# jamie8johnson/cqs

Measured on AMD Instinct MI355X. Metric: queries/sec @k=20 (brute-force cosine scan + top-k, 768-d fp32), higher is better.
Workload: dtype f32; 1 GPU; BASELINE configs[1]: 1000000 x 768 fp32 unit vectors, 1 query per step, brute-force cosine top-20; mode=single, rows_per_gpu=1000000, total_rows=1000000, dim=768, k=20, parallelism=single GPU, ranks_seen=1

## Files before the change

### cqs_amd/csrc/f32_score.h

```cpp
#pragma once
#include "scan_device.h"

namespace cqs {

template <int NCH, bool NT = false>
__device__ __forceinline__ void f32_row_fragments(const float* rp, uint32_t dim, uint32_t lane, f4 (&x)[NCH]) {
#pragma unroll
    for (int c = 0; c < NCH; ++c) {
        const uint32_t idx = (uint32_t)c * 256u + lane * 4u;
        const uint32_t off = idx < dim ? idx : dim - 4u;
        if (NT) x[c] = __builtin_nontemporal_load((const f4*)(rp + off));
        else x[c] = *(const f4*)(rp + off);
    }
}

template <int NCH>
__device__ __forceinline__ void f32_fragments(const float* rp, const float* qp, uint32_t dim, uint32_t lane, f4 (&x)[NCH],
                                              f4 (&qv)[NCH]) {
#pragma unroll
    for (int c = 0; c < NCH; ++c) {
        const uint32_t idx = (uint32_t)c * 256u + lane * 4u;
        const bool in = idx < dim;
        const uint32_t off = in ? idx : dim - 4u;
        x[c] = *(const f4*)(rp + off);
        const f4 v = *(const f4*)(qp + off);
        qv[c] = in ? v : (f4)(0.f);
    }
}

template <int NCH>
__device__ __forceinline__ float f32_dot_chain(const f4 (&x)[NCH], const f4 (&qv)[NCH]) {
    f2 acc2 = (f2)(0.f);
#pragma unroll
    for (int c = 0; c < NCH; ++c) {
        const f2 xlo = __builtin_shufflevector(x[c], x[c], 0, 1);
        const f2 xhi = __builtin_shufflevector(x[c], x[c], 2, 3);
        acc2 = __builtin_elementwise_fma(xlo, __builtin_shufflevector(qv[c], qv[c], 0, 1), acc2);
        acc2 = __builtin_elementwise_fma(xhi, __builtin_shufflevector(qv[c], qv[c], 2, 3), acc2);
    }
    float s = acc2.x + acc2.y;
#pragma unroll
    for (int m = 32; m >= 1; m >>= 1) s += __shfl_xor(s, m, 64);
    return s;
}

__device__ __forceinline__ bool f32_emit(float& s, uint32_t mode, float thr) {
    bool keep = __builtin_fabsf(s) <= 3.4028234664e38f;
    if (keep && mode == 1u) {
        s = s < 0.f ? 0.f : (s > 1.f ? 1.f : s);
        keep = s >= thr;
    }
    return keep;
}

}
```

### cqs_amd/csrc/index.hip

```cpp
#include <hip/hip_runtime.h>

#include <algorithm>
#include <cstdio>
#include <cstdlib>
#include <cstring>
#include <new>

#include "abi_guard.h"
#include "roctx.h"
#include "index_internal.h"
#include "scan_bf16.h"
#include "scan_i8.h"
#include "search_host.h"

using cqs::kMaxK;
using cqs::kRowsPerBlock;

namespace cqs_idx {

uint64_t pad_rows(uint64_t n) { return (n + kRowsPerBlock - 1) / kRowsPerBlock * kRowsPerBlock; }

int32_t fail(cqs_hip_index* idx, int32_t code, const char* what, hipError_t e) {
    char buf[512];
    if (e != hipSuccess)
// ... 148 lines not shown
    return CQS_HIP_OK;
}

void free_keep_tab(cqs_hip_index* x) {
    hipFree(x->d_keep_tab);
    hipHostFree(x->h_keep_tab);
    x->d_keep_tab = nullptr; x->h_keep_tab = nullptr; x->keep_tab_stride = 0;
}

bool ensure_keep_tab(cqs_hip_index* x) {
    const uint64_t cap = x->cap_rows > x->n ? x->cap_rows : x->n;
    const uint64_t stride = (cap + 31) / 32;
    if (x->d_keep_tab && x->keep_tab_stride >= stride) return true;
    if (stride > 0xFFFFFFFFull || quiesce(x) != hipSuccess) return false;
    free_keep_tab(x);
    const size_t bytes = (size_t)kCombineCap * stride * sizeof(uint32_t);
    if (hipMalloc(&x->d_keep_tab, bytes) != hipSuccess || hipHostMalloc(&x->h_keep_tab, bytes, hipHostMallocDefault) != hipSuccess) {
        (void)hipGetLastError();
        free_keep_tab(x);
        return false;
    }
    x->keep_tab_stride = stride;
    return true;
}

void read_combine_env(cqs_hip_index* x) {
    if (const char* ce = getenv("CQS_HIP_COMBINE")) x->combine = ce[0] != '0';
    if (const char* cf = getenv("CQS_HIP_COMBINE_FILTERED")) x->combine_filtered = cf[0] != '0';
    if (const char* ct = getenv("CQS_HIP_COMBINE_TAGGED")) x->combine_tagged = ct[0] != '0';
    x->cq.wait_us = cqs_combine::wait_us_from_env();
    if (const char* cb = getenv("CQS_HIP_COMBINE_BITS")) x->combine_relaxed = cb[0] == 'r';
}

int32_t create_common(uint64_t n, uint32_t dim, uint32_t metric, int32_t device, uint64_t row_base,
                      cqs_hip_index** out, cqs_hip_index** made) {
    if (!out) return CQS_HIP_ERR_INVALID;
    *out = nullptr;
    if (!cqs::scan_dim_supported(dim) || metric > CQS_HIP_METRIC_DOT) return CQS_HIP_ERR_INVALID;
    if (n + row_base > 0xFFFFFFFEull) return CQS_HIP_ERR_INVALID;
    int cnt = 0;
    if (hipGetDeviceCount(&cnt) != hipSuccess || cnt <= 0) return CQS_HIP_ERR_NO_DEVICE;
    if (device < 0 || device >= cnt) return CQS_HIP_ERR_INVALID;
    cqs_hip_index* x = new (std::nothrow) cqs_hip_index();
    if (!x) return CQS_HIP_ERR_NOMEM;
    x->device = device; x->n = n; x->dim = dim; x->metric = metric; x->row_base = row_base;
    if (hipSetDevice(device) != hipSuccess || hipStreamCreateWithFlags(&x->stream, hipStreamNonBlocking) != hipSuccess ||
        hipEventCreateWithFlags(&x->done, hipEventDisableTiming) != hipSuccess) {
        if (x->stream) hipStreamDestroy(x->stream);
        delete x;
        return CQS_HIP_ERR_DEVICE;
    }
    read_combine_env(x);
    if (getenv("CQS_HIP_DEBUG_STAMPS")) {
        const size_t bytes = (16 + 2 * cqs::kDbgWaves) * sizeof(unsigned long long);
        if (hipMalloc(&x->d_dbg, bytes) == hipSuccess) (void)hipMemset(x->d_dbg, 0, bytes);
    }
    hipDeviceProp_t prop;
    if (hipGetDeviceProperties(&prop, device) == hipSuccess && prop.multiProcessorCount > 0)
        x->n_cu = (uint32_t)prop.multiProcessorCount;
    *made = x;
    return CQS_HIP_OK;
}

}

using namespace cqs_idx;

extern "C" {

const char* cqs_hip_version(void) CQS_ABI_TRY { return "cqs-hip 0.1.0 (gfx950)"; } CQS_ABI_CATCH_VAL("cqs-hip")

int32_t cqs_hip_device_count(void) CQS_ABI_TRY {
    int cnt = 0;
    if (hipGetDeviceCount(&cnt) != hipSuccess) return 0;
    return cnt;
} CQS_ABI_CATCH_NOHANDLE

int32_t cqs_hip_device_mem(int32_t device, uint64_t* free_bytes, uint64_t* total_bytes) CQS_ABI_TRY {
    if (hipSetDevice(device) != hipSuccess) return CQS_HIP_ERR_NO_DEVICE;
    size_t f = 0, t = 0;
    if (hipMemGetInfo(&f, &t) != hipSuccess) return CQS_HIP_ERR_DEVICE;
    if (free_bytes) *free_bytes = f;
    if (total_bytes) *total_bytes = t;
    return CQS_HIP_OK;
} CQS_ABI_CATCH_NOHANDLE

}

int32_t cqs_idx::create_owned(const float* rows, uint64_t n, uint32_t dim, uint32_t metric, int32_t device,
                              uint64_t row_base, cqs_hip_index** out) {
    if (n > 0 && !rows) return CQS_HIP_ERR_INVALID;
    cqs_hip_index* x = nullptr;
    int32_t rc = create_common(n, dim, metric, device, row_base, out, &x);
    if (rc != CQS_HIP_OK) return rc;
    x->cap_rows = n ? n : 1;
    hipError_t e = hipMalloc(&x->d_rows, (size_t)x->cap_rows * dim * sizeof(float));
    if (e == hipSuccess && n)
        e = hipMemcpyAsync(x->d_rows, rows, (size_t)n * dim * sizeof(float), hipMemcpyHostToDevice, x->stream);
    if (e == hipSuccess) e = hipStreamSynchronize(x->stream);
    if (e != hipSuccess) {
        cqs_hip_index_destroy(x);
        return e == hipErrorOutOfMemory ? CQS_HIP_ERR_NOMEM : CQS_HIP_ERR_DEVICE;
    }
    *out = x;
    return CQS_HIP_OK;
}

// ... 466 lines not shown
```

### cqs_amd/csrc/index_shadow.hip

```cpp
#include <cstdlib>
#include <cstring>
#include <new>

#include "abi_guard.h"
#include "index_internal.h"
#include "scan_bf16.h"
#include "scan_fallback.h"
#include "scan_i8.h"

namespace cqs_idx {

constexpr uint64_t kShadowAutoBytes = 1ull << 30;
constexpr uint64_t kShadowFreeMinBytes = 4ull << 30;
constexpr double kShadowFreeFrac = 0.10;
constexpr uint32_t kStatWords = 12, kStatCounts = 3, kStatI8 = 5, kStatI8Counts = 8, kStatPrefix = 10;

struct Shadow {
    uint16_t* d_bf16 = nullptr;
    uint64_t cap = 0;
    int8_t* d_i8 = nullptr;
    float* d_i8_scale = nullptr;
    double r8 = 0.0, norm8 = 0.0;
    double r = 0.0;
    double norm = 0.0;
    unsigned long long* d_stats = nullptr;
    uint64_t* d_ekeys = nullptr;
    uint32_t* d_cert = nullptr;
    float* d_bq = nullptr;
    uint32_t* d_tickets = nullptr;
    uint64_t* d_fb_lists = nullptr;
    uint32_t* d_fb_tickets = nullptr;
    bool fb_one_launch = true;
    bool tail_prefix = true;
    uint8_t i8_groups = 2;
    uint32_t* h_cert = nullptr;
    uint32_t* h_cert_dev = nullptr;
};

static void shadow_device_counts(cqs_hip_index* x, uint32_t first, uint64_t* certified, uint64_t* fallbacks) {
    unsigned long long c[2];
    if (!x->shadow || !x->shadow->d_stats || quiesce(x) != hipSuccess) return;
    hipError_t e = hipMemcpyAsync(c, x->shadow->d_stats + first, sizeof c, hipMemcpyDeviceToHost, x->stream);
    if (e == hipSuccess) e = hipStreamSynchronize(x->stream);
    if (e != hipSuccess) { (void)hipGetLastError(); return; }
    *certified += c[0];
    *fallbacks += c[1];
}

static void i8_free(Shadow* s) {
    hipFree(s->d_i8); hipFree(s->d_i8_scale);
    s->d_i8 = nullptr; s->d_i8_scale = nullptr;
}

void shadow_free(cqs_hip_index* x) {
    Shadow* s = x->shadow;
    if (!s) return;
    uint64_t c = 0, f = 0;
    shadow_device_counts(x, kStatCounts, &c, &f);
    x->stat_certified.fetch_add(c, std::memory_order_relaxed);
    x->stat_fallbacks.fetch_add(f, std::memory_order_relaxed);
    c = f = 0;
    shadow_device_counts(x, kStatI8Counts, &c, &f);
    x->stat_i8_certified.fetch_add(c, std::memory_order_relaxed);
    x->stat_i8_fallbacks.fetch_add(f, std::memory_order_relaxed);
    i8_free(s);
    hipFree(s->d_bf16); hipFree(s->d_stats); hipFree(s->d_ekeys);
    hipFree(s->d_cert); hipFree(s->d_bq); hipFree(s->d_tickets); hipFree(s->d_fb_lists); hipFree(s->d_fb_tickets);
    hipHostFree(s->h_cert);
    delete s;
    x->shadow = nullptr;
}

ShadowBuffers shadow_buffers(const cqs_hip_index* x) {
    const Shadow* s = x->shadow;
    return s ? ShadowBuffers{s->d_bf16, s->d_i8, s->d_i8_scale} : ShadowBuffers{nullptr, nullptr, nullptr};
}

static int32_t shadow_convert(cqs_hip_index* x, uint64_t row0, bool* outlier) {
    Shadow* s = x->shadow;
    HIP_TRY(x, hipMemsetAsync(s->d_stats + 2, 0, sizeof(unsigned long long), x->stream));
    HIP_TRY(x, cqs::launch_shadow_build(x->d_rows, s->d_bf16, row0, x->n - row0, x->dim, cqs::shadow_gamma(x->dim),
                                        s->d_stats, x->stream));
    unsigned long long st[3];
    HIP_TRY(x, hipMemcpyAsync(st, s->d_stats, sizeof st, hipMemcpyDeviceToHost, x->stream));
    HIP_TRY(x, hipStreamSynchronize(x->stream));
    double r, m;
// ... 93 lines not shown
                hipFree(n8);
                i8_free(s);
                x->last_error = "extend: no device memory to grow the int8 copy of the shadow; int8 copy turned off";
            } else {
                e = hipMemcpyAsync(n8, s->d_i8, (size_t)n_old * x->dim, hipMemcpyDeviceToDevice, x->stream);
                if (e == hipSuccess) e = hipMemcpyAsync(ns, s->d_i8_scale, (size_t)n_old * sizeof(float), hipMemcpyDeviceToDevice, x->stream);
                if (e == hipSuccess) e = hipStreamSynchronize(x->stream);
                if (e != hipSuccess) { hipFree(n8); hipFree(ns); return fail(x, CQS_HIP_ERR_DEVICE, "extend: int8 copy", e); }
                i8_free(s);
                s->d_i8 = n8;
                s->d_i8_scale = ns;
            }
        }
        s->cap = x->cap_rows;
    }
    bool outlier = false;
    int32_t rc = shadow_convert(x, n_old, &outlier);
    if (rc == CQS_HIP_OK && s->d_i8 && !outlier) rc = i8_convert(x, n_old);
    if (rc != CQS_HIP_OK) return rc;
    if (outlier) {
        shadow_free(x);
        x->last_error = "extend: a new row has a component of magnitude >= 2^64; bf16 shadow turned off";
    }
    return CQS_HIP_OK;
}

static bool dim_ok(uint32_t dim) { return dim % 8u == 0u && dim <= cqs::kShadowMaxDim; }
static const char* const kDimRule = ": dim must be a multiple of 8 and <= 2048";

static int32_t shadow_enable(cqs_hip_index* x, const char* what) {
    std::string pre(what);
    if (!dim_ok(x->dim)) return fail(x, CQS_HIP_ERR_INVALID, (pre + kDimRule).c_str());
    if (x->shadow) return CQS_HIP_OK;
    auto oom = [&](hipError_t e) { (void)hipGetLastError(); shadow_free(x); return fail(x, CQS_HIP_ERR_NOMEM, (pre + ": allocation").c_str(), e); };
    Shadow* s = x->shadow = new (std::nothrow) Shadow();
    if (!s) return oom(hipErrorOutOfMemory);
    const uint64_t cap = x->cap_rows ? x->cap_rows : 1;
    hipError_t e;
    if ((e = hipMalloc(&s->d_bf16, (size_t)cap * x->dim * sizeof(uint16_t))) != hipSuccess) return oom(e);
    s->cap = cap;
    unsigned long long* stats = nullptr;
    if ((e = hipMalloc(&stats, kStatWords * sizeof(unsigned long long))) != hipSuccess) return oom(e);
    if ((e = hipMemsetAsync(stats, 0, kStatWords * sizeof(unsigned long long), x->stream)) != hipSuccess) { hipFree(stats); return oom(e); }
    s->d_stats = stats;
    if ((e = hipMalloc(&s->d_ekeys, (size_t)cqs::kShadowMaxQ * (cqs::kMaxK - 1) * sizeof(uint64_t))) != hipSuccess) return oom(e);
    if ((e = hipMalloc(&s->d_cert, (size_t)cqs::kShadowMaxQ * sizeof(uint32_t))) != hipSuccess) return oom(e);
    if ((e = hipMalloc(&s->d_bq, (size_t)cqs::kShadowMaxQ * sizeof(float))) != hipSuccess) return oom(e);
    if ((e = hipMalloc(&s->d_tickets, (size_t)cqs::kShadowMaxQ * sizeof(uint32_t))) != hipSuccess) return oom(e);
    if ((e = hipMemsetAsync(s->d_tickets, 0, (size_t)cqs::kShadowMaxQ * sizeof(uint32_t), x->stream)) != hipSuccess) return oom(e);
    const char* fb_env = getenv("CQS_HIP_FALLBACK_ONE_LAUNCH");
    s->fb_one_launch = !(fb_env && fb_env[0] == '0');
    const char* tp_env = getenv("CQS_HIP_TAIL_PREFIX");
    s->tail_prefix = !(tp_env && tp_env[0] == '0');
    const char* ig_env = getenv("CQS_HIP_I8_GROUPS");
    s->i8_groups = ig_env && ig_env[0] == '0' ? 0 : (ig_env && ig_env[0] == '1' ? 1 : 2);
    if ((e = hipMalloc(&s->d_fb_lists, cqs::f32_topk_fallback_words(x->n_cu) * sizeof(uint64_t))) != hipSuccess) return oom(e);
    if ((e = hipMalloc(&s->d_fb_tickets, (size_t)cqs::kMaxGemvQ * sizeof(uint32_t))) != hipSuccess) return oom(e);
    if ((e = hipMemsetAsync(s->d_fb_tickets, 0, (size_t)cqs::kMaxGemvQ * sizeof(uint32_t), x->stream)) != hipSuccess) return oom(e);
    if ((e = hipHostMalloc(&s->h_cert, (size_t)cqs::kShadowMaxQ * sizeof(uint32_t), hipHostMallocDefault)) != hipSuccess) return oom(e);
    if (hipHostGetDevicePointer((void**)&s->h_cert_dev, s->h_cert, 0) != hipSuccess) {
        (void)hipGetLastError();
        s->h_cert_dev = nullptr;
    }
    bool outlier = false;
    const int32_t rc = shadow_convert(x, 0, &outlier);
    if (rc != CQS_HIP_OK) { shadow_free(x); return rc; }
    if (outlier) {
        shadow_free(x);
        return fail(x, CQS_HIP_ERR_INVALID, (pre + ": a finite row has a component of magnitude >= 2^64").c_str());
    }
    return CQS_HIP_OK;
}

static bool i8_dim_ok(uint32_t dim) { return cqs::i8_dim_ok(dim); }
static const char* const kI8DimRule = ": dim must be a multiple of 16 and <= 2048";
static int32_t i8_auto(cqs_hip_index* x) {
    Shadow* s = x->shadow;
    if (!s || s->d_i8) return CQS_HIP_OK;
    const char* env = getenv("CQS_HIP_SCAN_I8");
    if (env && env[0] == '0') return CQS_HIP_OK;
    if (!(env && env[0] == '1') && x->n * x->dim * sizeof(float) < kShadowAutoBytes) return CQS_HIP_OK;
    const std::string pre("int8 copy of the shadow not built (the bf16 copy serves every block)");
    if (!i8_dim_ok(x->dim)) { x->last_error = pre + kI8DimRule; return CQS_HIP_OK; }
    size_t free_b = 0, total_b = 0;
    if (hipMemGetInfo(&free_b, &total_b) != hipSuccess) {
        (void)hipGetLastError();
        x->last_error = pre + ": hipMemGetInfo failed";
        return CQS_HIP_OK;
    }
    const uint64_t need = i8_bytes(s->cap, x->dim);
    const uint64_t frac = (uint64_t)(kShadowFreeFrac * (double)total_b);
    const uint64_t reserve = frac > kShadowFreeMinBytes ? frac : kShadowFreeMinBytes;
    bool built = false;
    if (free_b >= need && free_b - need >= reserve) {
        const int32_t rc = i8_enable(x, &built);
        if (rc != CQS_HIP_OK) return rc;
    }
    if (!built) x->last_error = pre + ": the device would keep less than max(4 GiB, 10 %) of its memory free with both copies";
    return CQS_HIP_OK;
}

int32_t shadow_auto(cqs_hip_index* x) {
    const char* env = getenv("CQS_HIP_SCAN_BF16");
    if (env && env[0] == '0') return CQS_HIP_OK;
    const bool any_size = env && env[0] == '1';
    const uint64_t f32_bytes = x->n * x->dim * sizeof(float);
// ... 15 lines not shown
    const uint64_t need = cap * x->dim * sizeof(uint16_t) + (cqs::kMaxK + 2ull) * cqs::kShadowMaxQ * sizeof(uint64_t) +
                          cqs::f32_topk_fallback_words(x->n_cu) * sizeof(uint64_t);
    const uint64_t frac = (uint64_t)(kShadowFreeFrac * (double)total_b);
    const uint64_t reserve = frac > kShadowFreeMinBytes ? frac : kShadowFreeMinBytes;
    if (free_b < need || free_b - need < reserve) {
        x->last_error = "bf16 shadow not built: the device would keep less than max(4 GiB, 10 %) of its memory free";
        return CQS_HIP_OK;
    }
    int32_t rc = shadow_enable(x, "bf16 shadow not built");
    if (rc == CQS_HIP_OK) rc = i8_auto(x);
    return rc == CQS_HIP_ERR_DEVICE ? rc : CQS_HIP_OK;
}

bool shadow_takes(const cqs_hip_index* x, uint32_t b, uint32_t k, bool gemv_only) {
    return x->shadow && b <= cqs::kShadowMaxQ && (gemv_only || !cqs::use_mfma(b, x->dim)) && cqs::shadow_kprime(k) >= k;
}

bool shadow_uses_i8(const cqs_hip_index* x, uint32_t b, uint32_t k) {
    return x->shadow && x->shadow->d_i8 && b <= cqs::kI8MaxQ && cqs::i8_k_ok(k);
}

static uint32_t shadow_group_tasks(const cqs_hip_index* x, bool i8, uint32_t kp) {
    const Shadow* s = x->shadow;
    if (!i8 || s->i8_groups == 0) return 1u;
    if (s->i8_groups == 1) return cqs::kMaxGroupTasks;
    const uint64_t kk = (uint64_t)kp + 1u;
    return 4u * kk * kk <= pad_rows(x->n) ? cqs::kMaxGroupTasks : 1u;
}

int32_t shadow_pass(cqs_hip_index* x, const float* d_q, uint32_t nb, uint32_t k, const uint32_t* d_keep, uint32_t mode,
                    float threshold, uint64_t* out_keys, uint32_t* out_counts, hipStream_t st, const uint32_t** device_gate,
                    const KeepTab* tab) {
    const Shadow* s = x->shadow;
    uint32_t* const cert = device_gate || !s->h_cert_dev ? s->d_cert : s->h_cert_dev;
    if (device_gate) *device_gate = cert;
    if (device_gate) HIP_TRY(x, order_after_last(x, st));
    const bool i8 = shadow_uses_i8(x, nb, k);
    const uint32_t kp = i8 ? cqs::i8_kprime(k) : cqs::shadow_kprime(k);
    const double r_max = i8 ? s->r8 : s->r, norm_max = i8 ? s->norm8 : s->norm;
    const bool bound_first = mode == CQS_HIP_MODE_PIPELINE;
    if (bound_first) {
        if (i8) HIP_TRY(x, cqs::launch_i8_bound(d_q, nb, x->dim, r_max, norm_max, s->d_bq, st));
        else HIP_TRY(x, cqs::launch_shadow_bound(d_q, nb, x->dim, r_max, norm_max, s->d_bq, st));
    }
    cqs::ScanArgs a = scan_args(x, d_q, nb, kp + 1u, d_keep, mode, threshold, i8 ? sizeof(int8_t) : sizeof(uint16_t), true, nullptr, nullptr, tab);
    a.group_tasks = shadow_group_tasks(x, i8, kp);
    const ShadowRows rows{i8 ? nullptr : s->d_bf16, i8 ? s->d_i8 : nullptr, s->d_i8_scale, s->d_bq};
    const int32_t rc = scan_select(x, a, st, &rows, nullptr, nullptr);
    if (rc == CQS_HIP_OK)
        HIP_TRY(x, cqs::launch_rescore_certify(a, (uint32_t)x->row_base, k, kp, bound_first ? 0u : (i8 ? 2u : 1u), r_max, norm_max,
                                               s->d_bq, s->d_tickets, s->d_ekeys, out_keys, out_counts, cert,
                                               device_gate ? s->d_stats + kStatCounts : nullptr,
                                               device_gate && i8 ? s->d_stats + kStatI8Counts : nullptr, s->tail_prefix,
                                               s->d_stats + kStatPrefix, x->d_dbg, st));
    return rc;
}

int32_t shadow_fallback(cqs_hip_index* x, const float* d_q, uint32_t nb, uint32_t k, const uint32_t* d_keep, uint32_t mode,
                        float threshold, uint64_t* out_keys, uint32_t* out_counts, hipStream_t st, const uint32_t* gate,
                        bool* taken) {
    const Shadow* s = x->shadow;
    *taken = false;
    if (!s || !gate || !s->fb_one_launch) return CQS_HIP_OK;
    const cqs::ScanArgs a = scan_args(x, d_q, nb, k, d_keep, mode, threshold, sizeof(float), false, nullptr, gate);
    if (!cqs::f32_topk_fallback_takes(a)) return CQS_HIP_OK;
    HIP_TRY(x, cqs::launch_f32_topk_fallback(a, (uint32_t)x->row_base, gate, s->d_fb_lists, s->d_fb_tickets, out_keys, out_counts, st));
    HIP_TRY(x, record_done(x, st));
    *taken = true;
    return CQS_HIP_OK;
}

hipError_t shadow_verdicts(cqs_hip_index* x, uint32_t nb, const uint32_t** h_cert) {
    const Shadow* s = x->shadow;
    *h_cert = s->h_cert;
    return s->h_cert_dev ? hipSuccess : hipMemcpyAsync(s->h_cert, s->d_cert, (size_t)nb * sizeof(uint32_t), hipMemcpyDeviceToHost, x->stream);
}

}

using namespace cqs_idx;

extern "C" {

int32_t cqs_hip_index_set_bf16_scan(cqs_hip_index* x, int32_t enable) CQS_ABI_TRY {
    if (!x || x->sh) return CQS_HIP_ERR_INVALID;
    std::lock_guard<std::mutex> g(x->mu);
    if (x->poisoned.load(std::memory_order_acquire)) return CQS_HIP_ERR_POISONED;
    HIP_TRY(x, hipSetDevice(x->device));
    HIP_TRY(x, quiesce(x));
    if (!enable) { shadow_free(x); return CQS_HIP_OK; }
    if (x->borrow) return fail(x, CQS_HIP_ERR_INVALID, "set_bf16_scan: index borrows its rows (they may change under the bound)");
    const int32_t rc = shadow_enable(x, "set_bf16_scan");
    return rc == CQS_HIP_OK ? i8_auto(x) : rc;
} CQS_ABI_CATCH(x)

void cqs_hip_index_bf16_stats(const cqs_hip_index* x, uint64_t* bytes, uint64_t* certified, uint64_t* fallbacks) CQS_ABI_TRY {
    uint64_t by = 0, c = 0, f = 0;
    if (x && !x->sh) {
        cqs_hip_index* m = const_cast<cqs_hip_index*>(x);
        std::lock_guard<std::mutex> g(m->mu);
        by = m->shadow ? m->shadow->cap * m->dim * sizeof(uint16_t) : 0;
        c = m->stat_certified.load(std::memory_order_relaxed);
        f = m->stat_fallbacks.load(std::memory_order_relaxed);
        if (m->shadow && hipSetDevice(m->device) == hipSuccess) shadow_device_counts(m, kStatCounts, &c, &f);
    }
    if (bytes) *bytes = by;
// ... 58 lines not shown
    for (uint32_t i = 0; i < b; ++i) {
        const float* q = queries + (size_t)i * x->dim;
        double s2 = 0.0;
        for (uint32_t d = 0; d < x->dim; ++d) s2 += (double)q[d] * (double)q[d];
        out_host[i] = cqs::i8_query_bound(s2, s->r8, s->norm8, x->dim);
    }
    return CQS_HIP_OK;
} CQS_ABI_CATCH(x)

int32_t cqs_hip_debug_shadow_bq(cqs_hip_index* x, uint32_t b, float* out) CQS_ABI_TRY {
    if (!x || x->sh || !out || b == 0) return CQS_HIP_ERR_INVALID;
    std::lock_guard<std::mutex> g(x->mu);
    const Shadow* s = x->shadow;
    if (!s || b > cqs::kShadowMaxQ) return CQS_HIP_ERR_INVALID;
    HIP_TRY(x, hipSetDevice(x->device));
    HIP_TRY(x, quiesce(x));
    HIP_TRY(x, hipMemcpyAsync(out, s->d_bq, (size_t)b * sizeof(float), hipMemcpyDeviceToHost, x->stream));
    HIP_TRY(x, hipStreamSynchronize(x->stream));
    return CQS_HIP_OK;
} CQS_ABI_CATCH(x)

int32_t cqs_hip_debug_shadow_tickets(cqs_hip_index* x, uint32_t b, uint32_t* out) CQS_ABI_TRY {
    if (!x || x->sh || !out || b == 0) return CQS_HIP_ERR_INVALID;
    std::lock_guard<std::mutex> g(x->mu);
    const Shadow* s = x->shadow;
    if (!s || b > cqs::kShadowMaxQ) return CQS_HIP_ERR_INVALID;
    HIP_TRY(x, hipSetDevice(x->device));
    HIP_TRY(x, quiesce(x));
    HIP_TRY(x, hipMemcpyAsync(out, s->d_tickets, (size_t)b * sizeof(uint32_t), hipMemcpyDeviceToHost, x->stream));
    HIP_TRY(x, hipStreamSynchronize(x->stream));
    return CQS_HIP_OK;
} CQS_ABI_CATCH(x)

int32_t cqs_hip_debug_tail_verdicts(cqs_hip_index* x, uint32_t b, uint32_t* out, uint64_t* out_prefix) CQS_ABI_TRY {
    if (!x || x->sh || !out || !out_prefix || b == 0) return CQS_HIP_ERR_INVALID;
    std::lock_guard<std::mutex> g(x->mu);
    const Shadow* s = x->shadow;
    if (!s || b > cqs::kShadowMaxQ) return CQS_HIP_ERR_INVALID;
    HIP_TRY(x, hipSetDevice(x->device));
    HIP_TRY(x, quiesce(x));
    HIP_TRY(x, hipMemcpyAsync(out, s->d_cert, (size_t)b * sizeof(uint32_t), hipMemcpyDeviceToHost, x->stream));
    HIP_TRY(x, hipMemcpyAsync(out_prefix, s->d_stats + kStatPrefix, 2 * sizeof(uint64_t), hipMemcpyDeviceToHost, x->stream));
    HIP_TRY(x, hipStreamSynchronize(x->stream));
    return CQS_HIP_OK;
} CQS_ABI_CATCH(x)

int32_t cqs_hip_debug_tail_stamps(cqs_hip_index* x, uint64_t* out) CQS_ABI_TRY {
    if (!x || x->sh || !out) return CQS_HIP_ERR_INVALID;
    std::lock_guard<std::mutex> g(x->mu);
    if (!x->d_dbg) return CQS_HIP_ERR_INVALID;
    HIP_TRY(x, hipSetDevice(x->device));
    HIP_TRY(x, quiesce(x));
    HIP_TRY(x, hipMemcpyAsync(out, x->d_dbg, 16 * sizeof(uint64_t), hipMemcpyDeviceToHost, x->stream));
    HIP_TRY(x, hipMemsetAsync(x->d_dbg, 0, 16 * sizeof(uint64_t), x->stream));
    HIP_TRY(x, hipStreamSynchronize(x->stream));
    return CQS_HIP_OK;
} CQS_ABI_CATCH(x)

int32_t cqs_hip_debug_shadow_stats(cqs_hip_index* x, double* out) CQS_ABI_TRY {
    if (!x || x->sh || !out) return CQS_HIP_ERR_INVALID;
    std::lock_guard<std::mutex> g(x->mu);
    const Shadow* s = x->shadow;
    if (!s) return CQS_HIP_ERR_INVALID;
    out[0] = s->r; out[1] = s->norm;
    out[2] = s->d_i8 ? s->r8 : 0.0; out[3] = s->d_i8 ? s->norm8 : 0.0;
    return CQS_HIP_OK;
} CQS_ABI_CATCH(x)

int32_t cqs_hip_debug_shadow_rows(cqs_hip_index* x, uint32_t copy, uint64_t row0, uint64_t rows, void* out, float* out_scales) CQS_ABI_TRY {
    if (!x || x->sh || !out || (copy != 1u && copy != 2u) || (copy == 2u && !out_scales)) return CQS_HIP_ERR_INVALID;
    std::lock_guard<std::mutex> g(x->mu);
    const Shadow* s = x->shadow;
    if (!s || (copy == 2u && !s->d_i8) || row0 > x->n || rows > x->n - row0) return CQS_HIP_ERR_INVALID;
    if (rows == 0) return CQS_HIP_OK;
    HIP_TRY(x, hipSetDevice(x->device));
    HIP_TRY(x, quiesce(x));
    if (copy == 1u) {
        HIP_TRY(x, hipMemcpyAsync(out, s->d_bf16 + row0 * x->dim, (size_t)rows * x->dim * sizeof(uint16_t), hipMemcpyDeviceToHost, x->stream));
    } else {
        HIP_TRY(x, hipMemcpyAsync(out, s->d_i8 + row0 * x->dim, (size_t)rows * x->dim, hipMemcpyDeviceToHost, x->stream));
        HIP_TRY(x, hipMemcpyAsync(out_scales, s->d_i8_scale + row0, (size_t)rows * sizeof(float), hipMemcpyDeviceToHost, x->stream));
    }
    HIP_TRY(x, hipStreamSynchronize(x->stream));
    return CQS_HIP_OK;
} CQS_ABI_CATCH(x)

int32_t cqs_hip_debug_shadow_scores(cqs_hip_index* x, uint32_t copy, const float* queries, uint32_t b, uint32_t k,
                                    const uint32_t* keep_bitset, uint32_t mode, float threshold, float* out_scores,
                                    float* out_bq) CQS_ABI_TRY {
    if (!x || x->sh || !queries || !out_scores || !out_bq || b == 0 || copy > 2u || mode > CQS_HIP_MODE_PIPELINE) return CQS_HIP_ERR_INVALID;
    if (k == 0 || k > cqs::kMaxK) return CQS_HIP_ERR_INVALID;
    std::lock_guard<std::mutex> g(x->mu);
    if (x->poisoned.load(std::memory_order_acquire)) return CQS_HIP_ERR_POISONED;
    const Shadow* s = x->shadow;
    if (!s || x->n == 0 || b > cqs::kMaxGemvQ || !shadow_takes(x, b, k, false)) return CQS_HIP_ERR_INVALID;
    if (copy == 2u && !(s->d_i8 && b <= cqs::kI8MaxQ && cqs::i8_k_ok(k))) return CQS_HIP_ERR_INVALID;
    HIP_TRY(x, hipSetDevice(x->device));
    HIP_TRY(x, quiesce(x));
    const bool i8 = copy == 2u || (copy == 0u && shadow_uses_i8(x, b, k));
    const uint32_t kp = copy == 2u ? cqs::i8_kprime(k) : cqs::shadow_kprime(k);
    const uint32_t k_scan = copy == 0u ? k : kp + 1u;
    int32_t rc = ensure_scratch(x, b, k_scan);
    if (rc != CQS_HIP_OK) return rc;
    const uint32_t* d_keep = nullptr;
    if (keep_bitset) {
        if ((rc = stage_keep(x, keep_bitset, (x->n + 31) / 32)) != CQS_HIP_OK) return rc;
        d_keep = x->d_keep;
// ... 24 lines not shown
```

### cqs_amd/csrc/scan_bf16.h

```cpp
#pragma once
#include <math.h>
#include <stdint.h>

#if defined(__HIPCC__)
#include <hip/hip_runtime.h>
#include "scan_kernels.h"
#define CQS_HD __host__ __device__
#else
#define CQS_HD
#endif

namespace cqs {

constexpr uint32_t kShadowMaxQ = 32;
constexpr uint32_t kShadowMaxDim = 2048;
constexpr uint32_t kShadowKMax = 1024;

inline uint32_t shadow_kprime(uint32_t k) {
    const uint32_t kp = 2u * k + 32u;
    return kp < kShadowKMax - 1u ? kp : kShadowKMax - 1u;
}

CQS_HD inline double shadow_gamma(uint32_t dim) {
    const double du = (double)dim * 0x1p-24;
    return du / (1.0 - du);
}

CQS_HD inline float round_up_f32(double v) {
    float f = (float)v;
    if ((double)f < v) f = nextafterf(f, INFINITY);
    return f;
}

CQS_HD inline float shadow_query_bound(double q_norm2, double r_max, double norm_max, uint32_t dim) {
    const double qn = sqrt(q_norm2) * (1.0 + 0x1p-40);
    if (!(qn * norm_max * (1.0 + shadow_gamma(dim)) < 0x1p100)) return INFINITY;
    return round_up_f32(qn * r_max * (1.0 + 0x1p-40) + (double)dim * 0x1p-140);
}

#if defined(__HIPCC__)
__device__ __forceinline__ double wave_q_norm2(const float* qp, uint32_t dim, uint32_t lane) {
    double s2 = 0.0;
    for (uint32_t d = lane; d < dim; d += 64u) s2 += (double)qp[d] * (double)qp[d];
#pragma unroll
    for (int m = 32; m >= 1; m >>= 1) s2 += __shfl_xor(s2, m, 64);
    return s2;
}
__device__ __forceinline__ float wave_shadow_bound(const float* qp, uint32_t dim, double r_max, double norm_max, uint32_t lane) {
    return shadow_query_bound(wave_q_norm2(qp, dim, lane), r_max, norm_max, dim);
}

hipError_t launch_shadow_build(const float* rows, uint16_t* shadow, uint64_t row0, uint64_t n_rows, uint32_t dim,
                               double gamma, unsigned long long* stats, hipStream_t st);

hipError_t launch_shadow_bound(const float* q, uint32_t b, uint32_t dim, double r_max, double norm_max, float* bq,
                               hipStream_t st);

hipError_t launch_scan_bf16(const ScanArgs& a, const uint16_t* shadow, const float* bq, hipStream_t st);

hipError_t launch_rescore_certify(const ScanArgs& a, uint32_t row_base, uint32_t k, uint32_t kprime, uint32_t bound,
                                  double r_max, double norm_max, float* bq, uint32_t* tickets, uint64_t* ekeys,
                                  uint64_t* out_keys, uint32_t* out_counts, uint32_t* cert, unsigned long long* counters,
                                  unsigned long long* counters2, bool prefix, unsigned long long* prefix_counts, unsigned long long* dbg,
                                  hipStream_t st);
#endif

}
```

### cqs_amd/csrc/scan_bf16.hip

```cpp
#include "scan_bf16.h"
#include "scan_i8.h"
#include "f32_score.h"
#include "launch_util.h"
#include "rank_sort.h"
#include "scan_gemv_device.h"
#include "select_device.h"
#include "shadow_build_device.h"
#include "tail_prefix.h"

namespace cqs {

static_assert(kShadowKMax == kMaxK, "shadow k' policy and the select agree on max k");

__device__ __forceinline__ float key_score(uint64_t key) {
    const uint32_t ok = (uint32_t)(key >> 32);
    return __uint_as_float((ok & 0x80000000u) ? (ok ^ 0x80000000u) : ~ok);
}

__global__ __launch_bounds__(256) void shadow_build_kernel(const float* __restrict__ rows, uint16_t* __restrict__ shadow,
                                                           uint64_t row0, uint64_t n_rows, uint32_t dim, double gamma,
                                                           unsigned long long* __restrict__ stats) {
    const int lane = threadIdx.x & 63;
    const uint64_t waves = (uint64_t)gridDim.x * (blockDim.x >> 6);
    for (uint64_t r = (uint64_t)blockIdx.x * (blockDim.x >> 6) + (threadIdx.x >> 6); r < n_rows; r += waves) {
        shadow_build_row(rows + (row0 + r) * dim, shadow + (row0 + r) * dim, dim, gamma, stats, lane);
    }
}

hipError_t launch_shadow_build(const float* rows, uint16_t* shadow, uint64_t row0, uint64_t n_rows, uint32_t dim,
                               double gamma, unsigned long long* stats, hipStream_t st) {
    if (n_rows == 0) return hipSuccess;
    const uint64_t blocks = (n_rows + 3u) / 4u;
    hipLaunchKernelGGL(shadow_build_kernel, dim3((uint32_t)(blocks < 8192u ? blocks : 8192u)), dim3(256), 0, st, rows,
                       shadow, row0, n_rows, dim, gamma, stats);
    return hipGetLastError();
}

__global__ __launch_bounds__(64) void shadow_bound_kernel(const float* __restrict__ q, uint32_t dim, double r_max,
                                                          double norm_max, float* __restrict__ bq) {
    const uint32_t lane = threadIdx.x;
    const float v = wave_shadow_bound(q + (size_t)blockIdx.x * dim, dim, r_max, norm_max, lane);
    if (lane == 0) bq[blockIdx.x] = v;
}

hipError_t launch_shadow_bound(const float* q, uint32_t b, uint32_t dim, double r_max, double norm_max, float* bq,
                               hipStream_t st) {
    if (b == 0) return hipSuccess;
    if (b > kShadowMaxQ) return hipErrorInvalidValue;
    hipLaunchKernelGGL(shadow_bound_kernel, dim3(b), dim3(64), 0, st, q, dim, r_max, norm_max, bq);
    return hipGetLastError();
}

struct Bf16ScanParams {
    const uint16_t* rows;
    uint32_t n, n_pad, dim;
    const float* q;
    float* scores;
    const uint32_t* keep;
    uint32_t mode;
    float thr;
// ... 208 lines not shown
            else if (left >= 4) { g = 4; e = launch_bf16<NCH, 4, 4, PQ>(a, shadow, bq, done, g, slot, st); }
            else if (left >= 2) { g = 2; e = launch_bf16<NCH, 2, 8, PQ>(a, shadow, bq, done, g, slot, st); }
            else { g = 1; e = launch_bf16<NCH, 1, 16, PQ>(a, shadow, bq, done, g, slot, st); }
        } else {
            if (left >= 2) { g = 2; e = launch_bf16<NCH, 2, 4, PQ>(a, shadow, bq, done, g, slot, st); }
            else { g = 1; e = launch_bf16<NCH, 1, 8, PQ>(a, shadow, bq, done, g, slot, st); }
        }
        if (e != hipSuccess) return e;
        done += g;
        slot = (slot + 1u) % kWorkWords;
    }
    return hipSuccess;
}

hipError_t launch_scan_bf16(const ScanArgs& a, const uint16_t* shadow, const float* bq, hipStream_t st) {
    if (a.b == 0 || a.n == 0) return hipSuccess;
    if (a.b > kShadowMaxQ || a.dim % 8u != 0u || a.dim > kShadowMaxDim || a.group_tasks != 1u) return hipErrorInvalidValue;
    if (a.keep_tab && !keep_tab_ok(a)) return hipErrorInvalidValue;
    switch ((a.dim + 511u) / 512u) {
        case 1: return a.keep_tab ? launch_bf16_groups<1, true>(a, shadow, bq, st) : launch_bf16_groups<1, false>(a, shadow, bq, st);
        case 2: return a.keep_tab ? launch_bf16_groups<2, true>(a, shadow, bq, st) : launch_bf16_groups<2, false>(a, shadow, bq, st);
        case 3: return a.keep_tab ? launch_bf16_groups<3, true>(a, shadow, bq, st) : launch_bf16_groups<3, false>(a, shadow, bq, st);
        case 4: return a.keep_tab ? launch_bf16_groups<4, true>(a, shadow, bq, st) : launch_bf16_groups<4, false>(a, shadow, bq, st);
        default: return hipErrorInvalidValue;
    }
}

struct TailParams {
    const float* rows;
    const float* q;
    uint32_t dim, k, kprime, mode, row_base;
    float thr;
    const float* scores;
    const float* gmax;
    const uint64_t* gaux;
    uint32_t n_pad;
    TaskTiers tiers;
    uint32_t group_tasks;
    uint32_t bins;
    uint32_t* work;
    uint64_t* ekeys;
    float* bq;
    uint32_t* tickets;
    uint32_t bound;
    double r_max, norm_max;
    uint64_t* out_keys;
    uint32_t* out_counts;
    uint32_t* cert;
    unsigned long long* counters;
    unsigned long long* counters2;
    uint32_t prefix;
    unsigned long long* prefix_counts;
    unsigned long long* dbg;
};

constexpr uint32_t kTailWaves = 16;

template <int NCH, bool DBG>
__global__ __launch_bounds__(1024) void rescore_certify_kernel(const TailParams p) {
    __shared__ uint64_t s_keys[kShadowKMax];
    __shared__ uint64_t s_sorted[kShadowKMax];
    __shared__ __attribute__((aligned(16))) uint32_t s_ok[kShadowKMax + 4];
    __shared__ uint32_t s_cnt, s_flag, s_last;
    const uint32_t lane = threadIdx.x & 63u;
    const uint32_t qi = blockIdx.y;
    const uint32_t wib = (uint32_t)__builtin_amdgcn_readfirstlane((int)(threadIdx.x >> 6));
    const uint32_t wave = blockIdx.x * kTailWaves + wib;
    const uint32_t n_waves = gridDim.x * kTailWaves;
    const uint32_t dim = p.dim;
    const float* qp = p.q + (size_t)qi * dim;
    unsigned long long* const dbg = DBG && qi == 0u ? p.dbg : nullptr;
#define CQS_TAIL_STAMP(i, who) do { if (DBG && dbg && (who)) dbg[i] = __builtin_amdgcn_s_memrealtime(); } while (0)
    if (threadIdx.x == 0) s_cnt = 0u;
    if (qi == 0u && blockIdx.x == 0u)
        for (uint32_t i = threadIdx.x; i < kWorkWords; i += 1024u) p.work[i] = 0u;
    const GroupMap map{p.tiers, p.group_tasks};
    const uint32_t n_groups = map.total();
    uint32_t found;
    const uint64_t* akeys = select_body(p.scores + (size_t)qi * p.n_pad, p.gmax + (size_t)qi * n_groups,
                                        p.gaux ? p.gaux + (size_t)qi * n_groups : nullptr, p.n_pad, map, p.kprime + 1u,
                                        p.row_base, p.bins, DBG ? dbg : nullptr, found);
    found = (uint32_t)__builtin_amdgcn_readfirstlane((int)found);
    const uint32_t ac = found < p.kprime + 1u ? found : p.kprime + 1u;
    const uint32_t nc = ac < p.kprime ? ac : p.kprime;
    const uint64_t key_next = ac > p.kprime ? akeys[p.kprime] : 0ull;

    auto write_out = [&](uint32_t m, bool ok) {
        const uint32_t k = p.k;
        const uint32_t outc = m < k ? m : k;
        for (uint32_t i = threadIdx.x; i < k; i += 1024u) p.out_keys[(size_t)qi * k + i] = (i < outc) ? s_sorted[i] : 0ull;
        if (threadIdx.x == 0) {
            p.out_counts[qi] = outc;
            p.cert[qi] = ok ? 1u : 0u;
            if (p.counters) atomicAdd(&p.counters[ok ? 0 : 1], 1ull);
            if (p.counters2) atomicAdd(&p.counters2[ok ? 0 : 1], 1ull);
        }
    };
    auto full_verdict = [&](uint32_t m, float bq) {
        bool ok = false;
        if (__builtin_fabsf(bq) <= 3.4028234664e38f) {
            if (ac <= p.kprime) ok = true;
            else if (m >= p.k) {
                float t = key_score(key_next) + bq;
                if (p.mode == 1u) t = t < 0.f ? 0.f : (t > 1.f ? 1.f : t);
                ok = t < key_score(s_sorted[p.k - 1u]);
            }
        }
        return ok;
    };

    for (uint32_t slot = wave; slot <= nc; slot += n_waves) {
        if (slot == 0u) {
            if (p.bound != 0u) {
                const float v = p.bound == 2u ? wave_i8_bound(qp, dim, p.r_max, p.norm_max, lane)
                                              : wave_shadow_bound(qp, dim, p.r_max, p.norm_max, lane);
                if (lane == 0u)
                    __hip_atomic_store((uint32_t*)p.bq + qi, __float_as_uint(v), __ATOMIC_RELAXED, __HIP_MEMORY_SCOPE_AGENT);
            }
            continue;
        }
        const uint32_t i = slot - 1u;
        const uint64_t key = akeys[i];
        const uint32_t grow = 0xFFFFFFFFu - (uint32_t)key;
        const float* rp = p.rows + (size_t)(grow - p.row_base) * dim;
        f4 x[NCH], qv[NCH];
        f32_fragments<NCH>(rp, qp, dim, lane, x, qv);
        CQS_TAIL_STAMP(6, slot == 1u && threadIdx.x == 64u);
        float s = f32_dot_chain<NCH>(x, qv);
        const bool keep = f32_emit(s, p.mode, p.thr);
        if (lane == 0u)
            __hip_atomic_store(p.ekeys + (size_t)qi * p.kprime + i, keep ? pack_key(okey(s), grow) : 0ull, __ATOMIC_RELAXED,
                               __HIP_MEMORY_SCOPE_AGENT);
        CQS_TAIL_STAMP(7, slot == 1u && threadIdx.x == 64u);
    }
    asm volatile("s_waitcnt vmcnt(0)" ::: "memory");
    __syncthreads();
    if (threadIdx.x == 0) {
        const uint32_t t = __hip_atomic_fetch_add(p.tickets + qi, 1u, __ATOMIC_RELAXED, __HIP_MEMORY_SCOPE_AGENT);
        const bool last = t == gridDim.x - 1u;
        if (last) __hip_atomic_store(p.tickets + qi, 0u, __ATOMIC_RELAXED, __HIP_MEMORY_SCOPE_AGENT);
        s_last = last ? 1u : 0u;
        CQS_TAIL_STAMP(10, blockIdx.x == 0u);
        CQS_TAIL_STAMP(14, last);
    }
    __syncthreads();
    if (s_last == 0u) return;

    const uint32_t j1 = p.prefix ? tail_prefix_first(p.k, nc) : nc;
    if (threadIdx.x < j1) {
        const uint64_t key = __hip_atomic_load(p.ekeys + (size_t)qi * p.kprime + threadIdx.x, __ATOMIC_RELAXED, __HIP_MEMORY_SCOPE_AGENT);
        if (key != 0ull) s_keys[atomicAdd(&s_cnt, 1u)] = key;
    }
    __syncthreads();
    CQS_TAIL_STAMP(11, threadIdx.x == 0u);
    uint32_t m = s_cnt;
    float bq = 0.f;
    if (threadIdx.x == 0) bq = __uint_as_float(__hip_atomic_load((uint32_t*)p.bq + qi, __ATOMIC_RELAXED, __HIP_MEMORY_SCOPE_AGENT));
    if (j1 < nc) rank_sort_keys_wide(s_keys, m, s_sorted, s_ok, &s_flag);
    else rank_sort_keys(s_keys, m, s_sorted, s_ok, &s_flag);
    if (j1 < nc) {
        if (threadIdx.x == 0) {
            bool ok = false;
            if (__builtin_fabsf(bq) <= 3.4028234664e38f && m >= p.k)
                ok = tail_prefix_certifies(akeys[j1], bq, p.mode, key_score(s_sorted[p.k - 1u]));
            s_last = ok ? 2u : 1u;
            if (p.prefix_counts) atomicAdd(&p.prefix_counts[ok ? 0 : 1], 1ull);
        }
        __syncthreads();
        if (s_last == 2u) {
            CQS_TAIL_STAMP(12, threadIdx.x == 0u);
            write_out(m, true);
            CQS_TAIL_STAMP(13, threadIdx.x == 0u);
            return;
        }
        if (threadIdx.x >= j1 && threadIdx.x < nc) {
            const uint64_t key = __hip_atomic_load(p.ekeys + (size_t)qi * p.kprime + threadIdx.x, __ATOMIC_RELAXED, __HIP_MEMORY_SCOPE_AGENT);
            if (key != 0ull) s_keys[atomicAdd(&s_cnt, 1u)] = key;
        }
        __syncthreads();
        m = s_cnt;
        rank_sort_keys(s_keys, m, s_sorted, s_ok, &s_flag);
    }
    CQS_TAIL_STAMP(12, threadIdx.x == 0u);
    bool ok = false;
    if (threadIdx.x == 0) ok = full_verdict(m, bq);
    write_out(m, ok);
    CQS_TAIL_STAMP(13, threadIdx.x == 0u);
#undef CQS_TAIL_STAMP
}

#ifndef CQS_TAIL_MAX_BLOCKS_PER_CU
#define CQS_TAIL_MAX_BLOCKS_PER_CU 1u
#endif

template <int NCH>
static void launch_tail(dim3 grid, dim3 block, hipStream_t st, const TailParams& tp) {
    if (tp.dbg) hipLaunchKernelGGL((rescore_certify_kernel<NCH, true>), grid, block, 0, st, tp);
    else hipLaunchKernelGGL((rescore_certify_kernel<NCH, false>), grid, block, 0, st, tp);
}

hipError_t launch_rescore_certify(const ScanArgs& a, uint32_t row_base, uint32_t k, uint32_t kprime, uint32_t bound,
                                  double r_max, double norm_max, float* bq, uint32_t* tickets, uint64_t* ekeys,
                                  uint64_t* out_keys, uint32_t* out_counts, uint32_t* cert, unsigned long long* counters,
                                  unsigned long long* counters2, bool prefix, unsigned long long* prefix_counts, unsigned long long* dbg,
                                  hipStream_t st) {
    const uint32_t b = a.b, dim = a.dim;
    if (b == 0) return hipSuccess;
    if (b > kShadowMaxQ || k == 0 || kprime < k || kprime >= kShadowKMax || a.k != kprime + 1u || dim % 8u != 0u ||
        dim > kShadowMaxDim || bound > 2u || (a.group_tasks != 1u && a.group_tasks != kMaxGroupTasks))
        return hipErrorInvalidValue;
    const TailParams tp{a.rows, a.q, dim, k, kprime, a.mode, row_base, a.threshold, a.scores, a.gmax, a.gaux, a.n_pad, a.tiers, a.group_tasks,
                        a.range_bins ? 2u : (a.linear_bins ? 1u : 0u), a.work, ekeys, bq, tickets, bound, r_max, norm_max,
                        out_keys, out_counts, cert, counters, counters2, prefix ? 1u : 0u, prefix_counts, dbg};
    const uint32_t want = (kprime + 1u + kTailWaves - 1u) / kTailWaves;
    uint32_t cap = a.n_cu * CQS_TAIL_MAX_BLOCKS_PER_CU / b;
    if (cap < 1u) cap = 1u;
    const dim3 grid(want < cap ? want : cap, b), block(64u * kTailWaves);
    switch ((dim + 255u) / 256u) {
        case 1: launch_tail<1>(grid, block, st, tp); break;
        case 2: launch_tail<2>(grid, block, st, tp); break;
        case 3: launch_tail<3>(grid, block, st, tp); break;
        case 4: launch_tail<4>(grid, block, st, tp); break;
        case 5: launch_tail<5>(grid, block, st, tp); break;
        case 6: launch_tail<6>(grid, block, st, tp); break;
        case 7: launch_tail<7>(grid, block, st, tp); break;
        case 8: launch_tail<8>(grid, block, st, tp); break;
        default: return hipErrorInvalidValue;
    }
    return hipGetLastError();
}

}
```

Baseline: 6873 queries/s.

## Rescore only the prefix candidates first, deferring the full tail to a slow path

Adds a tiered tail mode. The rescore/certify kernel first selects and rescores only the prefix candidates (first = tail_prefix_first(k, kprime)), and launches fewer workgroups sized to that prefix. Only when the prefix cannot certify the top-k does it rerun selection for the full kprime and rescore the remaining candidates in a batched loop inside the same kernel. The intent is to cut per-query tail work and launch width in the common case where the prefix certifies. The cost is a second select pass and serialized rescoring in one workgroup when certification fails. Adds batched fragment loads with sched barriers and extra debug stamp slots.

```diff
diff --git a/cqs_amd/csrc/f32_score.h b/cqs_amd/csrc/f32_score.h
--- a/cqs_amd/csrc/f32_score.h
+++ b/cqs_amd/csrc/f32_score.h
@@ -15,6 +15,16 @@
 }
 
 template <int NCH>
+__device__ __forceinline__ void f32_query_fragments(const float* qp, uint32_t dim, uint32_t lane, f4 (&qv)[NCH]) {
+#pragma unroll
+    for (int c = 0; c < NCH; ++c) {
+        const uint32_t idx = (uint32_t)c * 256u + lane * 4u;
+        const f4 v = *(const f4*)(qp + (idx < dim ? idx : dim - 4u));
+        qv[c] = idx < dim ? v : (f4)(0.f);
+    }
+}
+
+template <int NCH>
 __device__ __forceinline__ void f32_fragments(const float* rp, const float* qp, uint32_t dim, uint32_t lane, f4 (&x)[NCH],
                                               f4 (&qv)[NCH]) {
 #pragma unroll
@@ -26,6 +36,16 @@
         const f4 v = *(const f4*)(qp + off);
         qv[c] = in ? v : (f4)(0.f);
     }
+}
+
+template <int NCH>
+__device__ __forceinline__ void f32_fragments_batched(const float* rp, const float* qp, uint32_t dim, uint32_t lane, f4 (&x)[NCH],
+                                                      f4 (&qv)[NCH]) {
+    f32_row_fragments<NCH>(rp, dim, lane, x);
+    f32_row_fragments<NCH>(qp, dim, lane, qv);
+    __builtin_amdgcn_sched_barrier(0);
+#pragma unroll
+    for (int c = 0; c < NCH; ++c) qv[c] = (uint32_t)c * 256u + lane * 4u < dim ? qv[c] : (f4)(0.f);
 }
 
 template <int NCH>
diff --git a/cqs_amd/csrc/index.hip b/cqs_amd/csrc/index.hip
--- a/cqs_amd/csrc/index.hip
+++ b/cqs_amd/csrc/index.hip
@@ -224,7 +224,7 @@
     }
     read_combine_env(x);
     if (getenv("CQS_HIP_DEBUG_STAMPS")) {
-        const size_t bytes = (16 + 2 * cqs::kDbgWaves) * sizeof(unsigned long long);
+        const size_t bytes = (cqs::kDbgTailSlow + cqs::kDbgTailSlowWords) * sizeof(unsigned long long);
         if (hipMalloc(&x->d_dbg, bytes) == hipSuccess) (void)hipMemset(x->d_dbg, 0, bytes);
     }
     hipDeviceProp_t prop;
diff --git a/cqs_amd/csrc/index_shadow.hip b/cqs_amd/csrc/index_shadow.hip
--- a/cqs_amd/csrc/index_shadow.hip
+++ b/cqs_amd/csrc/index_shadow.hip
@@ -7,6 +7,7 @@
 #include "scan_bf16.h"
 #include "scan_fallback.h"
 #include "scan_i8.h"
+#include "tail_plan.h"
 
 namespace cqs_idx {
 
@@ -32,6 +33,7 @@
     uint32_t* d_fb_tickets = nullptr;
     bool fb_one_launch = true;
     bool tail_prefix = true;
+    uint8_t tail_first = 2;
     uint8_t i8_groups = 2;
     uint32_t* h_cert = nullptr;
     uint32_t* h_cert_dev = nullptr;
@@ -231,6 +233,8 @@
     s->fb_one_launch = !(fb_env && fb_env[0] == '0');
     const char* tp_env = getenv("CQS_HIP_TAIL_PREFIX");
     s->tail_prefix = !(tp_env && tp_env[0] == '0');
+    const char* tf_env = getenv("CQS_HIP_TAIL_PREFIX_FIRST");
+    s->tail_first = tf_env && tf_env[0] == '0' ? 0 : (tf_env && tf_env[0] == '1' ? 1 : 2);
     const char* ig_env = getenv("CQS_HIP_I8_GROUPS");
     s->i8_groups = ig_env && ig_env[0] == '0' ? 0 : (ig_env && ig_env[0] == '1' ? 1 : 2);
     if ((e = hipMalloc(&s->d_fb_lists, cqs::f32_topk_fallback_words(x->n_cu) * sizeof(uint64_t))) != hipSuccess) return oom(e);
@@ -352,6 +356,7 @@
                                                s->d_bq, s->d_tickets, s->d_ekeys, out_keys, out_counts, cert,
                                                device_gate ? s->d_stats + kStatCounts : nullptr,
                                                device_gate && i8 ? s->d_stats + kStatI8Counts : nullptr, s->tail_prefix,
+                                               s->tail_first == 2 ? cqs::tail_prefix_first_default(pad_rows(x->n), k) : s->tail_first == 1,
                                                s->d_stats + kStatPrefix, x->d_dbg, st));
     return rc;
 }
@@ -516,7 +521,9 @@
     HIP_TRY(x, hipSetDevice(x->device));
     HIP_TRY(x, quiesce(x));
     HIP_TRY(x, hipMemcpyAsync(out, x->d_dbg, 16 * sizeof(uint64_t), hipMemcpyDeviceToHost, x->stream));
+    HIP_TRY(x, hipMemcpyAsync(out + 16, x->d_dbg + cqs::kDbgTailSlow, cqs::kDbgTailSlowWords * sizeof(uint64_t), hipMemcpyDeviceToHost, x->stream));
     HIP_TRY(x, hipMemsetAsync(x->d_dbg, 0, 16 * sizeof(uint64_t), x->stream));
+    HIP_TRY(x, hipMemsetAsync(x->d_dbg + cqs::kDbgTailSlow, 0, cqs::kDbgTailSlowWords * sizeof(uint64_t), x->stream));
     HIP_TRY(x, hipStreamSynchronize(x->stream));
     return CQS_HIP_OK;
 } CQS_ABI_CATCH(x)
diff --git a/cqs_amd/csrc/scan_bf16.h b/cqs_amd/csrc/scan_bf16.h
--- a/cqs_amd/csrc/scan_bf16.h
+++ b/cqs_amd/csrc/scan_bf16.h
@@ -58,11 +58,13 @@
 
 hipError_t launch_scan_bf16(const ScanArgs& a, const uint16_t* shadow, const float* bq, hipStream_t st);
 
+constexpr uint32_t kDbgTailSlow = 16u + 2u * kDbgWaves;
+constexpr uint32_t kDbgTailSlowWords = 3u;
 hipError_t launch_rescore_certify(const ScanArgs& a, uint32_t row_base, uint32_t k, uint32_t kprime, uint32_t bound,
                                   double r_max, double norm_max, float* bq, uint32_t* tickets, uint64_t* ekeys,
                                   uint64_t* out_keys, uint32_t* out_counts, uint32_t* cert, unsigned long long* counters,
-                                  unsigned long long* counters2, bool prefix, unsigned long long* prefix_counts, unsigned long long* dbg,
-                                  hipStream_t st);
+                                  unsigned long long* counters2, bool prefix, bool prefix_first, unsigned long long* prefix_counts,
+                                  unsigned long long* dbg, hipStream_t st);
 #endif
 
 }
diff --git a/cqs_amd/csrc/scan_bf16.hip b/cqs_amd/csrc/scan_bf16.hip
--- a/cqs_amd/csrc/scan_bf16.hip
+++ b/cqs_amd/csrc/scan_bf16.hip
@@ -6,6 +6,7 @@
 #include "scan_gemv_device.h"
 #include "select_device.h"
 #include "shadow_build_device.h"
+#include "tail_plan.h"
 #include "tail_prefix.h"
 
 namespace cqs {
@@ -320,11 +321,10 @@
     uint32_t prefix;
     unsigned long long* prefix_counts;
     unsigned long long* dbg;
+    uint32_t first;
 };
 
-constexpr uint32_t kTailWaves = 16;
-
-template <int NCH, bool DBG>
+template <int NCH, bool DBG, bool TIER>
 __global__ __launch_bounds__(1024) void rescore_certify_kernel(const TailParams p) {
     __shared__ uint64_t s_keys[kShadowKMax];
     __shared__ uint64_t s_sorted[kShadowKMax];
@@ -344,14 +344,21 @@
         for (uint32_t i = threadIdx.x; i < kWorkWords; i += 1024u) p.work[i] = 0u;
     const GroupMap map{p.tiers, p.group_tasks};
     const uint32_t n_groups = map.total();
-    uint32_t found;
-    const uint64_t* akeys = select_body(p.scores + (size_t)qi * p.n_pad, p.gmax + (size_t)qi * n_groups,
-                                        p.gaux ? p.gaux + (size_t)qi * n_groups : nullptr, p.n_pad, map, p.kprime + 1u,
-                                        p.row_base, p.bins, DBG ? dbg : nullptr, found);
-    found = (uint32_t)__builtin_amdgcn_readfirstlane((int)found);
-    const uint32_t ac = found < p.kprime + 1u ? found : p.kprime + 1u;
-    const uint32_t nc = ac < p.kprime ? ac : p.kprime;
-    const uint64_t key_next = ac > p.kprime ? akeys[p.kprime] : 0ull;
+    const uint32_t first = TIER ? p.first : 0u;
+    uint32_t lim = TIER ? first : p.kprime;
+    uint32_t found, ac, nc;
+    uint64_t key_next;
+    const uint64_t* akeys;
+    auto run_select = [&](unsigned long long* stamps) {
+        akeys = select_body(p.scores + (size_t)qi * p.n_pad, p.gmax + (size_t)qi * n_groups,
+                            p.gaux ? p.gaux + (size_t)qi * n_groups : nullptr, p.n_pad, map, lim + 1u, p.row_base, p.bins,
+                            stamps, found);
+        found = (uint32_t)__builtin_amdgcn_readfirstlane((int)found);
+        ac = found < lim + 1u ? found : lim + 1u;
+        nc = ac < lim ? ac : lim;
+        key_next = ac > lim ? akeys[lim] : 0ull;
+    };
+    run_select(DBG ? dbg : nullptr);
 
     auto write_out = [&](uint32_t m, bool ok) {
         const uint32_t k = p.k;
@@ -392,7 +399,8 @@
         const uint32_t grow = 0xFFFFFFFFu - (uint32_t)key;
         const float* rp = p.rows + (size_t)(grow - p.row_base) * dim;
         f4 x[NCH], qv[NCH];
-        f32_fragments<NCH>(rp, qp, dim, lane, x, qv);
+        if constexpr (TIER) f32_fragments_batched<NCH>(rp, qp, dim, lane, x, qv);
+        else f32_fragments<NCH>(rp, qp, dim, lane, x, qv);
         CQS_TAIL_STAMP(6, slot == 1u && threadIdx.x == 64u);
         float s = f32_dot_chain<NCH>(x, qv);
         const bool keep = f32_emit(s, p.mode, p.thr);
@@ -415,6 +423,7 @@
     if (s_last == 0u) return;
 
     const uint32_t j1 = p.prefix ? tail_prefix_first(p.k, nc) : nc;
+    const bool proper = TIER ? found > first : j1 < nc;
     if (threadIdx.x < j1) {
         const uint64_t key = __hip_atomic_load(p.ekeys + (size_t)qi * p.kprime + threadIdx.x, __ATOMIC_RELAXED, __HIP_MEMORY_SCOPE_AGENT);
         if (key != 0ull) s_keys[atomicAdd(&s_cnt, 1u)] = key;
@@ -424,9 +433,9 @@
     uint32_t m = s_cnt;
     float bq = 0.f;
     if (threadIdx.x == 0) bq = __uint_as_float(__hip_atomic_load((uint32_t*)p.bq + qi, __ATOMIC_RELAXED, __HIP_MEMORY_SCOPE_AGENT));
-    if (j1 < nc) rank_sort_keys_wide(s_keys, m, s_sorted, s_ok, &s_flag);
+    if (proper) rank_sort_keys_wide(s_keys, m, s_sorted, s_ok, &s_flag);
     else rank_sort_keys(s_keys, m, s_sorted, s_ok, &s_flag);
-    if (j1 < nc) {
+    if (proper) {
         if (threadIdx.x == 0) {
             bool ok = false;
             if (__builtin_fabsf(bq) <= 3.4028234664e38f && m >= p.k)
@@ -441,11 +450,39 @@
             CQS_TAIL_STAMP(13, threadIdx.x == 0u);
             return;
         }
-        if (threadIdx.x >= j1 && threadIdx.x < nc) {
-            const uint64_t key = __hip_atomic_load(p.ekeys + (size_t)qi * p.kprime + threadIdx.x, __ATOMIC_RELAXED, __HIP_MEMORY_SCOPE_AGENT);
-            if (key != 0ull) s_keys[atomicAdd(&s_cnt, 1u)] = key;
+        if constexpr (!TIER) {
+            if (threadIdx.x >= j1 && threadIdx.x < nc) {
+                const uint64_t key = __hip_atomic_load(p.ekeys + (size_t)qi * p.kprime + threadIdx.x, __ATOMIC_RELAXED, __HIP_MEMORY_SCOPE_AGENT);
+                if (key != 0ull) s_keys[atomicAdd(&s_cnt, 1u)] = key;
+            }
+        } else {
+            CQS_TAIL_STAMP(kDbgTailSlow + 0u, threadIdx.x == 0u);
+            lim = p.kprime;
+            run_select(nullptr);
+            CQS_TAIL_STAMP(kDbgTailSlow + 1u, threadIdx.x == 0u);
+            constexpr int kRU = NCH <= 3 ? 4 : (NCH <= 4 ? 3 : (NCH <= 6 ? 2 : 1));
+            f4 qv[NCH];
+            f32_query_fragments<NCH>(qp, dim, lane, qv);
+            for (uint32_t i0 = first + wib * (uint32_t)kRU; i0 < nc; i0 += kTailWaves * (uint32_t)kRU) {
+                f4 x[kRU][NCH];
+                uint32_t grow[kRU];
+#pragma unroll
+                for (int u = 0; u < kRU; ++u) {
+                    const uint32_t i = i0 + (uint32_t)u < nc ? i0 + (uint32_t)u : nc - 1u;
+                    grow[u] = 0xFFFFFFFFu - (uint32_t)akeys[i];
+                    f32_row_fragments<NCH>(p.rows + (size_t)(grow[u] - p.row_base) * dim, dim, lane, x[u]);
+                }
+                __builtin_amdgcn_sched_barrier(0);
+#pragma unroll
+                for (int u = 0; u < kRU; ++u) {
+                    float s = f32_dot_chain<NCH>(x[u], qv);
+                    const bool keep = f32_emit(s, p.mode, p.thr);
+                    if (lane == 0u && i0 + (uint32_t)u < nc && keep) s_keys[atomicAdd(&s_cnt, 1u)] = pack_key(okey(s), grow[u]);
+                }
+            }
         }
         __syncthreads();
+        if constexpr (TIER) CQS_TAIL_STAMP(kDbgTailSlow + 2u, threadIdx.x == 0u);
         m = s_cnt;
         rank_sort_keys(s_keys, m, s_sorted, s_ok, &s_flag);
     }
@@ -463,27 +500,30 @@
 
 template <int NCH>
 static void launch_tail(dim3 grid, dim3 block, hipStream_t st, const TailParams& tp) {
-    if (tp.dbg) hipLaunchKernelGGL((rescore_certify_kernel<NCH, true>), grid, block, 0, st, tp);
-    else hipLaunchKernelGGL((rescore_certify_kernel<NCH, false>), grid, block, 0, st, tp);
+    if (tp.first != 0u) {
+        if (tp.dbg) hipLaunchKernelGGL((rescore_certify_kernel<NCH, true, true>), grid, block, 0, st, tp);
+        else hipLaunchKernelGGL((rescore_certify_kernel<NCH, false, true>), grid, block, 0, st, tp);
+    } else {
+        if (tp.dbg) hipLaunchKernelGGL((rescore_certify_kernel<NCH, true, false>), grid, block, 0, st, tp);
+        else hipLaunchKernelGGL((rescore_certify_kernel<NCH, false, false>), grid, block, 0, st, tp);
+    }
 }
 
 hipError_t launch_rescore_certify(const ScanArgs& a, uint32_t row_base, uint32_t k, uint32_t kprime, uint32_t bound,
                                   double r_max, double norm_max, float* bq, uint32_t* tickets, uint64_t* ekeys,
                                   uint64_t* out_keys, uint32_t* out_counts, uint32_t* cert, unsigned long long* counters,
-                                  unsigned long long* counters2, bool prefix, unsigned long long* prefix_counts, unsigned long long* dbg,
-                                  hipStream_t st) {
+                                  unsigned long long* counters2, bool prefix, bool prefix_first, unsigned long long* prefix_counts,
+                                  unsigned long long* dbg, hipStream_t st) {
     const uint32_t b = a.b, dim = a.dim;
     if (b == 0) return hipSuccess;
     if (b > kShadowMaxQ || k == 0 || kprime < k || kprime >= kShadowKMax || a.k != kprime + 1u || dim % 8u != 0u ||
         dim > kShadowMaxDim || bound > 2u || (a.group_tasks != 1u && a.group_tasks != kMaxGroupTasks))
         return hipErrorInvalidValue;
+    const uint32_t first = tail_plan_first(k, kprime, prefix, prefix_first);
     const TailParams tp{a.rows, a.q, dim, k, kprime, a.mode, row_base, a.threshold, a.scores, a.gmax, a.gaux, a.n_pad, a.tiers, a.group_tasks,
                         a.range_bins ? 2u : (a.linear_bins ? 1u : 0u), a.work, ekeys, bq, tickets, bound, r_max, norm_max,
-                        out_keys, out_counts, cert, counters, counters2, prefix ? 1u : 0u, prefix_counts, dbg};
-    const uint32_t want = (kprime + 1u + kTailWaves - 1u) / kTailWaves;
-    uint32_t cap = a.n_cu * CQS_TAIL_MAX_BLOCKS_PER_CU / b;
-    if (cap < 1u) cap = 1u;
-    const dim3 grid(want < cap ? want : cap, b), block(64u * kTailWaves);
+                        out_keys, out_counts, cert, counters, counters2, prefix ? 1u : 0u, prefix_counts, dbg, first};
+    const dim3 grid(tail_plan_workgroups(tail_plan_slots(kprime, first), b, a.n_cu, CQS_TAIL_MAX_BLOCKS_PER_CU), b), block(64u * kTailWaves);
     switch ((dim + 255u) / 256u) {
         case 1: launch_tail<1>(grid, block, st, tp); break;
         case 2: launch_tail<2>(grid, block, st, tp); break;
diff --git a/cqs_amd/csrc/tail_plan.h b/cqs_amd/csrc/tail_plan.h
--- /dev/null
+++ b/cqs_amd/csrc/tail_plan.h
@@ -0,0 +1,26 @@
+#pragma once
+#include "tail_prefix.h"
+
+namespace cqs {
+
+constexpr uint32_t kTailWaves = 16;
+
+CQS_TP_HD inline uint32_t tail_plan_first(uint32_t k, uint32_t kprime, bool prefix, bool prefix_first) {
+    if (!prefix || !prefix_first) return 0u;
+    const uint32_t j1 = tail_prefix_first(k, kprime);
+    return j1 < kprime ? j1 : 0u;
+}
+
+CQS_TP_HD inline uint32_t tail_plan_slots(uint32_t kprime, uint32_t first) { return (first ? first : kprime) + 1u; }
+
+CQS_TP_HD inline uint32_t tail_plan_workgroups(uint32_t slots, uint32_t b, uint32_t n_cu, uint32_t per_cu) {
+    const uint32_t want = (slots + kTailWaves - 1u) / kTailWaves;
+    uint32_t cap = b ? n_cu * per_cu / b : 0u;
+    if (cap < 1u) cap = 1u;
+    return want < cap ? want : cap;
+}
+
+constexpr uint64_t kTailFirstMaxRows = 4ull << 20;
+CQS_TP_HD inline bool tail_prefix_first_default(uint64_t n_pad, uint32_t ) { return n_pad <= kTailFirstMaxRows; }
+
+}
```

Result: faster. 7008 queries/s (median of 6 runs) (+2.0%).
